# thunlp/OpenMatch

Hardware: NVIDIA H100
Metric: queries/sec top-1000 over 8.8M x 768 corpus (higher is better)
Workload: dtype f16

## Files before the change

openmatch_b200/csrc/scan_gemm.cuh:

```cuda
#pragma once
#include <cuda_fp16.h>

#include "scan_epilogue.cuh"

namespace om {

constexpr int kScanBlockN = 256;
constexpr int kScanStages = 3;
constexpr int kScanABytes = kBlockM * kBlockK * 2;
constexpr int kScanBBytes = kScanBlockN * kBlockK * 2;
constexpr int kScanStageBytes = kScanABytes + kScanBBytes;
constexpr int kScanConsumers = 256;
constexpr int kScanStash = 4;
constexpr int kScanStashOffset = kScanStages * kScanStageBytes;
constexpr int kScanStashBytes = 2 * 2 * kScanStash * kScanConsumers * 8;
constexpr int kScanBarOffset = kScanStashOffset + kScanStashBytes;
constexpr int kScanSmemBytes = kScanBarOffset + 2 * kScanStages * 8 + 1024;
static_assert(kScanSmemBytes <= 232448, "scan ring + stash exceed the 227 KB of shared memory an H100 block may use");

template <int H>
__device__ __forceinline__ float scan_pick(const float (&acc)[128], int i) {
  float a[32], b[16], c[8], d[4], e[2];
#pragma unroll
  for (int j = 0; j < 32; ++j) a[j] = (i & 1) ? acc[4 * j + 2 * H + 1] : acc[4 * j + 2 * H];
#pragma unroll
  for (int j = 0; j < 16; ++j) b[j] = (i & 2) ? a[2 * j + 1] : a[2 * j];
#pragma unroll
  for (int j = 0; j < 8; ++j) c[j] = (i & 4) ? b[2 * j + 1] : b[2 * j];
#pragma unroll
  for (int j = 0; j < 4; ++j) d[j] = (i & 8) ? c[2 * j + 1] : c[2 * j];
#pragma unroll
  for (int j = 0; j < 2; ++j) e[j] = (i & 16) ? d[2 * j + 1] : d[2 * j];
  return (i & 32) ? e[1] : e[0];
}

template <int H>
__device__ __forceinline__ int scan_filter_row(const float (&acc)[128], float t, int row, int lim, int q4, int col0,
                                               unsigned long long* stash, unsigned long long* cand, int* count,
                                               int* overflow, int C, uint32_t row_base) {
  float mx = acc[2 * H];
#pragma unroll
  for (int j = 0; j < 32; ++j) mx = fmaxf(mx, fmaxf(acc[4 * j + 2 * H], acc[4 * j + 2 * H + 1]));
  if (!(mx > t)) return 0;
  uint32_t lo = 0, hi = 0;
#pragma unroll
  for (int i = 0; i < 32; ++i) {
    lo |= (acc[4 * (i >> 1) + 2 * H + (i & 1)] > t ? 1u : 0u) << i;
    hi |= (acc[4 * (16 + (i >> 1)) + 2 * H + (i & 1)] > t ? 1u : 0u) << i;
  }
  unsigned long long mask = (static_cast<unsigned long long>(hi) << 32) | lo;
  if (lim < kScanBlockN) {
#pragma unroll 1
    for (int i = 0; i < 64; ++i)
      if (8 * (i >> 1) + 2 * q4 + (i & 1) >= lim) mask &= ~(1ull << i);
  }
  const int n = __popcll(mask);
  int pos = 0;
  if (n > kScanStash) {
    pos = atomicAdd(count + row, n - kScanStash);
    if (pos + (n - kScanStash) > C) *overflow = 1;
  }
  unsigned long long* mine = cand + static_cast<size_t>(row) * C;
  int idx = 0;
#pragma unroll 1
  while (mask) {
    const int i = __ffsll(static_cast<long long>(mask)) - 1;
    mask &= mask - 1;
    const unsigned long long key =
        make_key(scan_pick<H>(acc, i), row_base + static_cast<uint32_t>(col0 + 8 * (i >> 1) + 2 * q4 + (i & 1)));
    if (idx < kScanStash)
      stash[idx * kScanConsumers] = key;
    else if (pos + idx - kScanStash < C)
      mine[pos + idx - kScanStash] = key;
    ++idx;
  }
  return n < kScanStash ? n : kScanStash;
}

template <int CQ, int CX>
struct ScanCluster {
  static_assert((CQ == 2 || CQ == 4) && (CX == 1 || CX == 2), "scan cluster shapes: CQ in {2, 4}, CX in {1, 2}");
  static constexpr int kSize = CQ * CX;
  static constexpr int kShare = CQ + CX - 1;
  static constexpr int kQRows = kBlockM / CX;
  static constexpr int kXRows = kScanBlockN / CQ;
  static constexpr int kEmptyArrivals = kShare * (kScanConsumers / 32);
  __device__ static uint32_t peer_rank(uint32_t rank, int j) {
    const uint32_t a = rank % CQ, b = rank / CQ;
    if (j < CQ - 1) {
      const uint32_t o = static_cast<uint32_t>(j);
      return (o < a ? o : o + 1) + CQ * b;
    }
    const uint32_t o = static_cast<uint32_t>(j - (CQ - 1));
    return a + CQ * (o < b ? o : o + 1);
  }
  __device__ static uint16_t q_mask(uint32_t rank) {
    uint32_t m = 0;
#pragma unroll
    for (int b = 0; b < CX; ++b) m |= 1u << (rank % CQ + CQ * b);
    return static_cast<uint16_t>(m);
  }
  __device__ static uint16_t x_mask(uint32_t rank) {
    return static_cast<uint16_t>(((1u << CQ) - 1u) << (CQ * (rank / CQ)));
  }
};

template <int CQ, int CX>
__global__ void __launch_bounds__(kGemmProducerThreads + kScanConsumers, 1)
scan_wide_kernel(const __grid_constant__ CUtensorMap tmQ, const __grid_constant__ CUtensorMap tmX, int K,
                 const float* __restrict__ thr, unsigned long long* cand, int* count, int* overflow, int nq, int n_cols,
                 int C, uint32_t row_base) {
  using Cl = ScanCluster<CQ, CX>;
  extern __shared__ uint8_t smem_raw[];
  uint8_t* smem = reinterpret_cast<uint8_t*>((reinterpret_cast<uintptr_t>(smem_raw) + 1023) & ~uintptr_t(1023));
  unsigned long long* stash = reinterpret_cast<unsigned long long*>(smem + kScanStashOffset);
  uint64_t* full_bar = reinterpret_cast<uint64_t*>(smem + kScanBarOffset);
  uint64_t* empty_bar = full_bar + kScanStages;
  const uint32_t rank = cluster_ctarank();
  const int qa = static_cast<int>(rank % CQ), xb = static_cast<int>(rank / CQ);
  const int warp = __shfl_sync(0xffffffffu, static_cast<int>(threadIdx.x >> 5), 0);
  const int lane = static_cast<int>(threadIdx.x & 31);

  if (warp == 0 && lane == 0) {
    tma_prefetch_desc(&tmQ);
    tma_prefetch_desc(&tmX);
  }
  if (warp == 1 && lane == 0) {
    ring_init(full_bar, empty_bar, kScanStages, Cl::kEmptyArrivals);
    fence_barrier_init();
  }
  cluster_sync_all();

  const int qgroups = (nq + CQ * kBlockM - 1) / (CQ * kBlockM);
  const int num_tiles = qgroups * ((n_cols + CX * kScanBlockN - 1) / (CX * kScanBlockN));
  const int num_k = (K + kBlockK - 1) / kBlockK;

  if (warp < 4) {
    setmaxnreg_dec<40>();
    if (warp == 0 && lane == 0) {
      const uint16_t qmask = Cl::q_mask(rank), xmask = Cl::x_mask(rank);
      Ring<kScanStages> ring;
      for (int tile = static_cast<int>(cluster_id_x()); tile < num_tiles; tile += static_cast<int>(cluster_count_x())) {
        const int m_blk = (tile % qgroups) * CQ + qa;
        const int n_blk = (tile / qgroups) * CX + xb;
        for (int kb = 0; kb < num_k; ++kb) {
          uint64_t* bar = ring_acquire_tx(full_bar, empty_bar, ring, kScanStageBytes, 30);
          uint8_t* sa = smem + ring.stage * kScanStageBytes;
          if constexpr (CX == 1)
            tma_load_2d(sa, &tmQ, bar, kb * kBlockK, m_blk * kBlockM);
          else
            tma_load_2d_multicast(sa + xb * (Cl::kQRows * kBlockK * 2), &tmQ, bar, kb * kBlockK,
                                  m_blk * kBlockM + xb * Cl::kQRows, qmask);
          tma_load_2d_multicast(sa + kScanABytes + qa * (Cl::kXRows * kBlockK * 2), &tmX, bar, kb * kBlockK,
                                n_blk * kScanBlockN + qa * Cl::kXRows, xmask);
          ring.advance();
        }
      }
    }
  } else {
    setmaxnreg_inc<232>();
    const int et = static_cast<int>(threadIdx.x) - kGemmProducerThreads;
    const int wg = et >> 7;
    const int q4 = lane & 3;
    const int frow = 64 * wg + 16 * (warp & 3) + (lane >> 2);
    Ring<kScanStages> ring;
    int buf = 0;
    int p_n0 = 0, p_n1 = 0, p_excl0 = 0, p_excl1 = 0, p_pos0 = 0, p_pos1 = 0, p_row = 0, p_buf = 0;
    auto drain = [&]() {
      if (!__any_sync(0xffffffffu, (p_n0 | p_n1) != 0)) return;
      const int b0 = __shfl_sync(0xffffffffu, p_pos0, lane & ~3) + p_excl0;
      const int b1 = __shfl_sync(0xffffffffu, p_pos1, lane & ~3) + p_excl1;
      const unsigned long long* s = stash + p_buf * (2 * kScanStash * kScanConsumers) + et;
      unsigned long long* m0 = cand + static_cast<size_t>(p_row) * C;
      unsigned long long* m1 = cand + static_cast<size_t>(p_row + 8) * C;
      for (int j = 0; j < p_n0; ++j)
        if (b0 + j < C) m0[b0 + j] = s[j * kScanConsumers];
      for (int j = 0; j < p_n1; ++j)
        if (b1 + j < C) m1[b1 + j] = s[(kScanStash + j) * kScanConsumers];
      if ((p_n0 > 0 && b0 + p_n0 > C) || (p_n1 > 0 && b1 + p_n1 > C)) *overflow = 1;
      p_n0 = p_n1 = 0;
    };

    uint32_t peers[Cl::kShare - 1];
#pragma unroll
    for (int j = 0; j < Cl::kShare - 1; ++j) peers[j] = Cl::peer_rank(rank, j);
    auto release = [&](uint32_t s) {
      if (lane == 0) {
        mbar_arrive(&empty_bar[s]);
#pragma unroll
        for (int j = 0; j < Cl::kShare - 1; ++j) mbar_arrive_remote(&empty_bar[s], peers[j]);
      }
    };

    for (int tile = static_cast<int>(cluster_id_x()); tile < num_tiles; tile += static_cast<int>(cluster_count_x())) {
      const int m_blk = (tile % qgroups) * CQ + qa;
      const int n_blk = (tile / qgroups) * CX + xb;
      const int row0 = m_blk * kBlockM + frow, row1 = row0 + 8;
      const float inf = __int_as_float(0x7f800000);
      const float t0 = row0 < nq ? thr[row0] : inf, t1 = row1 < nq ? thr[row1] : inf;

      float acc[128];
#pragma unroll
      for (int i = 0; i < 128; ++i) acc[i] = 0.f;
      ring_consume(
          full_bar, ring, 0, num_k, 31,
          [&](uint32_t stage, uint32_t accumulate) {
            const uint32_t a_addr = smem_u32(smem + stage * kScanStageBytes) + wg * (64 * 128);
            const uint32_t b_addr = smem_u32(smem + stage * kScanStageBytes + kScanABytes);
#pragma unroll
            for (int k = 0; k < kBlockK / kWgmmaK; ++k)
              wgmma_m64n256k16_f16<0, 0>(acc, wgmma_desc(a_addr + k * 32, kDescKMajorSW128),
                                         wgmma_desc(b_addr + k * 32, kDescKMajorSW128), (accumulate | k) != 0 ? 1u : 0u);
          },
          release);
      wgmma_fence_regs(acc);

      drain();
      const int col0 = n_blk * kScanBlockN;
      const int lim = n_cols - col0;
      unsigned long long* sb = stash + buf * (2 * kScanStash * kScanConsumers) + et;
      const int k0 = scan_filter_row<0>(acc, t0, row0, lim, q4, col0, sb, cand, count, overflow, C, row_base);
      const int k1 = scan_filter_row<1>(acc, t1, row1, lim, q4, col0, sb + kScanStash * kScanConsumers, cand, count,
                                        overflow, C, row_base);
      if (__any_sync(0xffffffffu, (k0 | k1) != 0)) {
        int x0 = k0, x1 = k1;
        int y0 = __shfl_up_sync(0xffffffffu, x0, 1, 4), y1 = __shfl_up_sync(0xffffffffu, x1, 1, 4);
        if (q4 >= 1) x0 += y0, x1 += y1;
        y0 = __shfl_up_sync(0xffffffffu, x0, 2, 4), y1 = __shfl_up_sync(0xffffffffu, x1, 2, 4);
        if (q4 >= 2) x0 += y0, x1 += y1;
        const int n0 = __shfl_sync(0xffffffffu, x0, lane | 3), n1 = __shfl_sync(0xffffffffu, x1, lane | 3);
        if (q4 == 0) {
          if (n0 > 0) p_pos0 = atomicAdd(count + row0, n0);
          if (n1 > 0) p_pos1 = atomicAdd(count + row1, n1);
        }
        p_n0 = k0;
        p_n1 = k1;
        p_excl0 = x0 - k0;
        p_excl1 = x1 - k1;
        p_row = row0;
        p_buf = buf;
        buf ^= 1;
      }
    }
    drain();
  }

  __syncthreads();
  cluster_sync_all();
}

template <int CQ, int CX>
static inline cudaError_t scan_wide_max_clusters(int num_sms, int* out) {
  static int max_clusters = -1;
  if (max_clusters < 0) {
    constexpr int kSize = ScanCluster<CQ, CX>::kSize;
    cudaError_t e =
        cudaFuncSetAttribute(scan_wide_kernel<CQ, CX>, cudaFuncAttributeMaxDynamicSharedMemorySize, kScanSmemBytes);
    if (e != cudaSuccess) return e;
    cudaLaunchConfig_t cfg = {};
    cfg.gridDim = dim3(kSize * (num_sms / kSize));
    cfg.blockDim = dim3(kGemmProducerThreads + kScanConsumers);
    cfg.dynamicSmemBytes = kScanSmemBytes;
    cudaLaunchAttribute attr[1];
    attr[0].id = cudaLaunchAttributeClusterDimension;
    attr[0].val.clusterDim = {static_cast<unsigned>(kSize), 1, 1};
    cfg.attrs = attr;
    cfg.numAttrs = 1;
    int n = 0;
    e = cudaOccupancyMaxActiveClusters(&n, scan_wide_kernel<CQ, CX>, &cfg);
    if (e != cudaSuccess) return e;
    max_clusters = n < num_sms / kSize ? n : num_sms / kSize;
  }
  *out = max_clusters;
  return cudaSuccess;
}

template <int CQ, int CX>
static inline cudaError_t launch_scan_wide(const __half* Q, int64_t ldq, const __half* X, int64_t ldx, int nq, int n_cols,
                                           int K, const float* thr, unsigned long long* cand, int* count, int* overflow,
                                           int C, uint32_t row_base, int num_sms, cudaStream_t stream) {
  using Cl = ScanCluster<CQ, CX>;
  CUtensorMap tmQ, tmX;
  if (make_tmap_bf16_2d(&tmQ, Q, (uint64_t)K, (uint64_t)nq, (uint64_t)ldq * 2, kBlockK, Cl::kQRows) != 0)
    return cudaErrorInvalidValue;
  if (make_tmap_bf16_2d(&tmX, X, (uint64_t)K, (uint64_t)n_cols, (uint64_t)ldx * 2, kBlockK, Cl::kXRows) != 0)
    return cudaErrorInvalidValue;
  int max_clusters = 0;
  cudaError_t e = scan_wide_max_clusters<CQ, CX>(num_sms, &max_clusters);
  if (e != cudaSuccess) return e;
  if (max_clusters < 1) return cudaErrorNotSupported;
  cudaLaunchConfig_t cfg = {};
  cfg.blockDim = dim3(kGemmProducerThreads + kScanConsumers);
  cfg.dynamicSmemBytes = kScanSmemBytes;
  cfg.stream = stream;
  cudaLaunchAttribute attr[1];
  attr[0].id = cudaLaunchAttributeClusterDimension;
  attr[0].val.clusterDim = {static_cast<unsigned>(Cl::kSize), 1, 1};
  cfg.attrs = attr;
  cfg.numAttrs = 1;
  const int qgroups = (nq + CQ * kBlockM - 1) / (CQ * kBlockM);
  const int64_t num_tiles = static_cast<int64_t>(qgroups) * ((n_cols + CX * kScanBlockN - 1) / (CX * kScanBlockN));
  const int clusters = num_tiles < max_clusters ? static_cast<int>(num_tiles) : max_clusters;
  cfg.gridDim = dim3(Cl::kSize * clusters);
  return cudaLaunchKernelEx(&cfg, scan_wide_kernel<CQ, CX>, tmQ, tmX, K, thr, cand, count, overflow, nq, n_cols, C,
                            row_base);
}

static inline cudaError_t launch_scan_cluster(int cq, int cx, const __half* Q, int64_t ldq, const __half* X, int64_t ldx,
                                              int nq, int n_cols, int K, const float* thr, unsigned long long* cand,
                                              int* count, int* overflow, int C, uint32_t row_base, int num_sms,
                                              cudaStream_t stream) {
  if (nq <= 0 || n_cols <= 0 || K <= 0) return cudaSuccess;
  if (cq == 2 && cx == 1)
    return launch_scan_wide<2, 1>(Q, ldq, X, ldx, nq, n_cols, K, thr, cand, count, overflow, C, row_base, num_sms, stream);
  if (cq == 4 && cx == 1)
    return launch_scan_wide<4, 1>(Q, ldq, X, ldx, nq, n_cols, K, thr, cand, count, overflow, C, row_base, num_sms, stream);
  if (cq == 2 && cx == 2)
    return launch_scan_wide<2, 2>(Q, ldq, X, ldx, nq, n_cols, K, thr, cand, count, overflow, C, row_base, num_sms, stream);
  if (cq == 4 && cx == 2)
    return launch_scan_wide<4, 2>(Q, ldq, X, ldx, nq, n_cols, K, thr, cand, count, overflow, C, row_base, num_sms, stream);
  return cudaErrorInvalidValue;
}

static inline cudaError_t scan_cluster_capacity(int cq, int cx, int num_sms, int* out) {
  *out = -1;
  if (cq == 2 && cx == 1) return scan_wide_max_clusters<2, 1>(num_sms, out);
  if (cq == 4 && cx == 1) return scan_wide_max_clusters<4, 1>(num_sms, out);
  if (cq == 2 && cx == 2) return scan_wide_max_clusters<2, 2>(num_sms, out);
  if (cq == 4 && cx == 2) return scan_wide_max_clusters<4, 2>(num_sms, out);
  return cudaSuccess;
}

}
```

openmatch_b200/csrc/search.cu:

```cuda
#include <cuda_fp16.h>
#include <float.h>
#include <math.h>
#include <stdlib.h>
#include <string.h>

#include <algorithm>
#include <new>
#include <type_traits>
#include <vector>

#include "common.h"
#include "gemm.cuh"
#include "nccl_dyn.h"
#include "quant_i8.cuh"
#include "scan_epilogue.cuh"
#include "scan_gemm.cuh"
#include "scan_i8.cuh"

namespace om {

__device__ __forceinline__ void bitonic_sort_desc(unsigned long long* s, int P, int tid, int nthreads) {
  for (int k = 2; k <= P; k <<= 1) {
    for (int j = k >> 1; j > 0; j >>= 1) {
      for (int t = tid; t < (P >> 1); t += nthreads) {
// ... 621 lines not shown
  __half* xh = nullptr;
  int8_t* xq = nullptr;
  float* gstats = nullptr;
  bool gstats_stale = false;
  int64_t st_nonfinite = 0;
  int64_t rescore_slack = -1;
  int force_safe = 0;
  int pair_scan = 1;
  int scan_cq = 0, scan_cx = 0;
  int growth = 0;
  int certify = 1;
  int exact_only = 0;
  int stage_scores = 0;
  int64_t st_rounds = 0, st_retries = 0, st_capacity = 0, st_launches = 0;
  int64_t st_flagged = 0, st_flagged_wide = 0, st_exact = 0;
  int64_t st_scan_cluster = 0, st_scan_clusters = 0;
  int profile = 0;
  double st_scan_us = 0, st_select_us = 0, st_final_us = 0, st_other_us = 0;
  std::vector<cudaEvent_t> ev;
  std::vector<int> ev_kind;
  size_t ev_used = 0;
  DevBuf ws, ows, sws;
  int* h_status = nullptr;
};

template <typename F>
static decltype(auto) with_rows(const om_index* ix, F&& f) {
  switch (ix->storage) {
    case OM_I8: return f(ix->xq);
    case OM_F16: return f(ix->xh);
    default: return f(ix->xf);
  }
}

template <typename RowT>
static int64_t pitch_of(const RowT*, int d) { return StoredRow<RowT>::pitch(d); }

struct RowBuf {
  void** p;
  size_t row_bytes;
  const char* name;
};
template <typename RowT>
static RowBuf row_buf(RowT** p, int d, const char* name) {
  return {reinterpret_cast<void**>(p), StoredRow<RowT>::pitch(d) * sizeof(RowT), name};
}

static int index_grow(om_index* ix, int64_t need) {
  if (need <= ix->cap) return 0;
  int64_t ncap = std::max<int64_t>(need, ix->cap + ix->cap / 2);
  ncap = round_up(std::max<int64_t>(ncap, 1024), 256);
  std::vector<RowBuf> bufs;
  switch (ix->storage) {
    case OM_I8: bufs = {row_buf(&ix->xq, ix->d, "int8")}; break;
    case OM_F16: bufs = {row_buf(&ix->xh, ix->d, "fp16")}; break;
    default: bufs = {row_buf(&ix->xf, ix->d, "fp32"), row_buf(&ix->xh, ix->d, "fp16")};
  }
  void* fresh[2] = {};
  OM_CUDA(cudaDeviceSynchronize());
  for (size_t b = 0; b < bufs.size(); ++b) {
    if (dev_malloc(&fresh[b], static_cast<size_t>(ncap) * bufs[b].row_bytes) != cudaSuccess) {
      for (void* p : fresh) cudaFree(p);
      cudaGetLastError();
      return fail(OM_ENOMEM, "index: cannot allocate the %s rows for %lld rows", bufs[b].name, (long long)ncap);
    }
    if (ix->n > 0)
      OM_CUDA(cudaMemcpy(fresh[b], *bufs[b].p, static_cast<size_t>(ix->n) * bufs[b].row_bytes, cudaMemcpyDeviceToDevice));
  }
  OM_CUDA(cudaDeviceSynchronize());
  for (size_t b = 0; b < bufs.size(); ++b) {
    cudaFree(*bufs[b].p);
    *bufs[b].p = fresh[b];
  }
  ix->cap = ncap;
  return 0;
}

static inline int grid_for(int64_t n, int threads) {
  int64_t g = (n + threads - 1) / threads;
  return static_cast<int>(std::min<int64_t>(std::max<int64_t>(g, 1), 132 * 16));
}

static int settle_reset(om_index* ix, cudaStream_t st) {
  if (!ix->gstats_stale) return 0;
  OM_CUDA(cudaMemsetAsync(ix->gstats, 0, 3 * sizeof(float), st));
  ix->gstats_stale = false;
  return 0;
}

static int stage_input(const void* x, om_memkind kind, size_t bytes, cudaStream_t st, const void** src, void** tmp) {
  *src = x;
  if (kind != OM_HOST) return 0;
  OM_CUDA(cudaMalloc(tmp, bytes));
  OM_CUDA(cudaMemcpyAsync(*tmp, x, bytes, cudaMemcpyHostToDevice, st));
  *src = *tmp;
  return 0;
}

template <typename F>
static decltype(auto) with_input(const void* src, om_dtype dtype, F&& f) {
  if (dtype == OM_F32) return f(static_cast<const float*>(src));
  if (dtype == OM_BF16) return f(static_cast<const __nv_bfloat16*>(src));
  return f(static_cast<const __half*>(src));
}

extern "C" {

int om_index_create(int d, om_index** out) { return om_index_create_typed(d, OM_F32, out); }

int om_index_create_typed(int d, om_dtype storage, om_index** out) {
  if (!out || d <= 0) return fail(OM_EINVAL, "om_index_create: d must be positive");
  if (storage != OM_F32 && storage != OM_F16 && storage != OM_I8)
    return fail(OM_EINVAL, "om_index_create_typed: storage must be OM_F32, OM_F16 or OM_I8");
  OM_TRY(device_sm_count());
  om_index* ix = new (std::nothrow) om_index();
  if (!ix) return fail(OM_ENOMEM, "om_index_create: out of host memory");
  ix->d = d;
  ix->dpad = storage == OM_I8 ? i8_dpad(d) : StoredRow<__half>::pitch(d);
  ix->storage = storage;
  if (cudaMalloc(&ix->gstats, 4 * sizeof(float)) != cudaSuccess || cudaMemset(ix->gstats, 0, 4 * sizeof(float)) != cudaSuccess ||
      cudaHostAlloc(&ix->h_status, 8 * sizeof(int), cudaHostAllocDefault) != cudaSuccess) {
    cudaGetLastError();
    cudaFree(ix->gstats);
    delete ix;
    return fail(OM_ENOMEM, "om_index_create: cannot allocate index state");
  }
  *out = ix;
  return 0;
}

void om_index_destroy(om_index* ix) {
  if (!ix) return;
  cudaFree(ix->xf);
  cudaFree(ix->xh);
  cudaFree(ix->xq);
  cudaFree(ix->gstats);
  if (ix->h_status) cudaFreeHost(ix->h_status);
  ix->ws.release();
  ix->ows.release();
  ix->sws.release();
  for (cudaEvent_t e : ix->ev) cudaEventDestroy(e);
  delete ix;
}

int64_t om_index_ntotal(const om_index* ix) { return ix ? ix->n : 0; }
int om_index_dim(const om_index* ix) { return ix ? ix->d : 0; }
int om_index_storage(const om_index* ix) { return ix ? ix->storage : fail(OM_EINVAL, "om_index_storage: null index"); }

int om_index_reset(om_index* ix) {
  if (!ix) return fail(OM_EINVAL, "om_index_reset: null index");
  ix->n = 0;
  ix->gstats_stale = true;
  ix->st_nonfinite = 0;
  return 0;
}

int om_index_reserve_rows(om_index* ix, int64_t n, void** dev_rows, int64_t* row_pitch_elems) {
  if (!ix || n < 0 || !dev_rows || !row_pitch_elems) return fail(OM_EINVAL, "om_index_reserve_rows: bad arguments");
  if (ix->n + n > 0xfffffff0ll) return fail(OM_EINVAL, "index shard limited to 2^32-16 rows; shard the corpus");
  OM_TRY(index_grow(ix, ix->n + n));
  with_rows(ix, [&](auto* xs) {
    *row_pitch_elems = pitch_of(xs, ix->d);
    *dev_rows = xs + ix->n * *row_pitch_elems;
  });
  return 0;
}

int om_index_reserve(om_index* ix, int64_t n, float** dev_rows) {
  if (!ix || n < 0 || !dev_rows) return fail(OM_EINVAL, "om_index_reserve: bad arguments");
  if (ix->storage != OM_F32)
    return fail(OM_ESTATE, "om_index_reserve: the index stores %s rows; use om_index_reserve_rows",
                ix->storage == OM_F16 ? "fp16" : "int8");
  void* rows = nullptr;
  int64_t pitch = 0;
  OM_TRY(om_index_reserve_rows(ix, n, &rows, &pitch));
  *dev_rows = static_cast<float*>(rows);
  return 0;
}

int om_index_commit(om_index* ix, int64_t n, void* stream) {
  if (!ix || n < 0 || ix->n + n > ix->cap) return fail(OM_EINVAL, "om_index_commit: more rows than reserved");
  if (n == 0) return 0;
  cudaStream_t st = static_cast<cudaStream_t>(stream);
  OM_TRY(settle_reset(ix, st));
  with_rows(ix, [&](auto* xs) {
    auto* rows = xs + ix->n * pitch_of(xs, ix->d);
    if constexpr (std::is_same<decltype(rows), float*>::value)
      rows_to_f16_kernel<<<grid_for(n, 8), 256, 0, st>>>(rows, ix->xh + static_cast<size_t>(ix->n) * ix->dpad, n, ix->d,
                                                         ix->dpad, nullptr, nullptr, ix->gstats);
    else
      commit_rows_kernel<<<grid_for(n, 8), 256, 0, st>>>(rows, n, ix->d, ix->gstats, reinterpret_cast<int*>(ix->gstats) + 2);
  });
  OM_CUDA(cudaGetLastError());
  ix->n += n;
  return 0;
}

static int add_converted(om_index* ix, const void* x, om_memkind kind, om_dtype dtype, int64_t n, cudaStream_t st) {
  void* rows = nullptr;
  int64_t pitch = 0;
  OM_TRY(om_index_reserve_rows(ix, n, &rows, &pitch));
  const size_t elems = static_cast<size_t>(n) * ix->d;
  const void* src = nullptr;
  void* tmp = nullptr;
  OM_TRY(stage_input(x, kind, elems * (dtype == OM_F32 ? 4 : 2), st, &src, &tmp));
  const bool i8 = ix->storage == OM_I8;
  int* bad = reinterpret_cast<int*>(ix->gstats) + 3;
  cudaError_t e = cudaMemsetAsync(bad, 0, sizeof(int), st);
  if (e == cudaSuccess)
    e = with_input(src, dtype, [&](const auto* in) {
      if (i8)
        quantize_rows_i8_kernel<<<grid_for(n, 8), 256, 0, st>>>(in, n, ix->d, static_cast<int8_t*>(rows), pitch, bad);
      else
        to_f16_rows_kernel<<<grid_for(static_cast<int64_t>(elems), 256), 256, 0, st>>>(in, n, ix->d, static_cast<__half*>(rows),
                                                                                        ix->dpad, bad);
      return cudaGetLastError();
    });
  if (e == cudaSuccess) e = cudaMemcpyAsync(ix->h_status + 4, bad, sizeof(int), cudaMemcpyDeviceToHost, st);
  if (e == cudaSuccess) e = cudaStreamSynchronize(st);
  if (tmp) cudaFree(tmp);
  OM_CUDA(e);
  if (ix->h_status[4] > 0 && i8)
    return fail(OM_EINVAL, "om_index_add: %d rows hold inf or NaN; int8 storage cannot hold them and no row was added",
                ix->h_status[4]);
  if (ix->h_status[4] > 0)
    return fail(OM_EINVAL, "om_index_add: %d elements are NaN or round to +-inf in fp16 (|x| >= 65520); fp16 storage cannot "
                "hold them and no row was added", ix->h_status[4]);
  return om_index_commit(ix, n, st);
}

int om_index_add(om_index* ix, const void* x, om_memkind kind, om_dtype dtype, int64_t n, void* stream) {
  if (!ix || (!x && n > 0) || n < 0) return fail(OM_EINVAL, "om_index_add: bad arguments");
  if (n == 0) return 0;
  if (dtype != OM_F32 && dtype != OM_BF16 && dtype != OM_F16) return fail(OM_EINVAL, "om_index_add: unsupported dtype %d", (int)dtype);
  cudaStream_t st = static_cast<cudaStream_t>(stream);
  if (ix->storage != OM_F32) return add_converted(ix, x, kind, dtype, n, st);
  float* dst = nullptr;
  OM_TRY(om_index_reserve(ix, n, &dst));
  const size_t elems = static_cast<size_t>(n) * ix->d;
  const void* src = x;
  void* tmp = nullptr;
  if (dtype != OM_F32) OM_TRY(stage_input(x, kind, elems * 2, st, &src, &tmp));
  OM_TRY(with_input(src, dtype, [&](const auto* in) -> int {
    if constexpr (std::is_same<decltype(in), const float*>::value) {
      OM_CUDA(cudaMemcpyAsync(dst, in, elems * 4, kind == OM_HOST ? cudaMemcpyHostToDevice : cudaMemcpyDeviceToDevice, st));
    } else {
      to_f32<<<grid_for(elems, 256), 256, 0, st>>>(in, dst, (int64_t)elems);
      OM_CUDA(cudaGetLastError());
    }
    return 0;
  }));
  if (tmp) {
    OM_CUDA(cudaStreamSynchronize(st));
    cudaFree(tmp);
  }
  OM_TRY(om_index_commit(ix, n, stream));
  if (kind == OM_HOST) OM_CUDA(cudaStreamSynchronize(st));
  return 0;
}

int om_index_set_param(om_index* ix, const char* name, int64_t value) {
  if (!ix || !name) return fail(OM_EINVAL, "om_index_set_param: bad arguments");
  if (!strcmp(name, "rescore_slack")) {
    ix->rescore_slack = value;
  } else if (!strcmp(name, "force_safe_rounds")) {
    ix->force_safe = value != 0;
  } else if (!strcmp(name, "round_growth")) {
    if (value != 0 && (value < 2 || value > 8)) return fail(OM_EINVAL, "round_growth must be 0 (auto) or in [2, 8]");
    ix->growth = static_cast<int>(value);
  } else if (!strcmp(name, "pair_scan")) {
    ix->pair_scan = value != 0;
  } else if (!strcmp(name, "scan_cluster_q")) {
    if (value != 0 && value != 2 && value != 4) return fail(OM_EINVAL, "scan_cluster_q must be 0 (auto), 2 or 4");
    ix->scan_cq = static_cast<int>(value);
  } else if (!strcmp(name, "scan_cluster_x")) {
    if (value != 0 && value != 1 && value != 2) return fail(OM_EINVAL, "scan_cluster_x must be 0 (auto), 1 or 2");
    ix->scan_cx = static_cast<int>(value);
  } else if (!strcmp(name, "profile")) {
    ix->profile = static_cast<int>(value);
  } else if (!strcmp(name, "certify")) {
    ix->certify = value != 0;
  } else if (!strcmp(name, "exact_only")) {
    ix->exact_only = value != 0;
  } else if (!strcmp(name, "debug_stage_scores")) {
    ix->stage_scores = value != 0;
  } else {
    return fail(OM_EINVAL, "om_index_set_param: unknown parameter '%s'", name);
  }
  return 0;
}

int64_t om_index_get_stat(const om_index* ix, const char* name) {
  if (!ix || !name) return -1;
  if (!strcmp(name, "rounds")) return ix->st_rounds;
  if (!strcmp(name, "overflow_retries")) return ix->st_retries;
  if (!strcmp(name, "candidates")) return ix->st_capacity;
  if (!strcmp(name, "launches")) return ix->st_launches;
  if (!strcmp(name, "uncertified")) return ix->st_flagged;
  if (!strcmp(name, "uncertified_wide")) return ix->st_flagged_wide;
  if (!strcmp(name, "exact_queries")) return ix->st_exact;
  if (!strcmp(name, "nonfinite_rows")) return ix->st_nonfinite;
  if (!strcmp(name, "scan_cluster")) return ix->st_scan_cluster;
  if (!strcmp(name, "scan_max_clusters")) return ix->st_scan_clusters;
  if (!strcmp(name, "scan_ns")) return static_cast<int64_t>(ix->st_scan_us * 1e3);
  if (!strcmp(name, "select_ns")) return static_cast<int64_t>(ix->st_select_us * 1e3);
  if (!strcmp(name, "finalize_ns")) return static_cast<int64_t>(ix->st_final_us * 1e3);
  if (!strcmp(name, "other_ns")) return static_cast<int64_t>(ix->st_other_us * 1e3);
  return -1;
}

}

namespace {

struct Timed {
  om_index* ix;
  cudaStream_t st;
  bool on;
  Timed(om_index* ix_, cudaStream_t st_, int kind) : ix(ix_), st(st_), on(ix_->profile != 0) {
    static const char* nvtx_names[4] = {"om.search.scan", "om.search.select", "om.search.rescore", "om.search.exchange_certify"};
    nvtxRangePushA(nvtx_names[kind & 3]);
    if (!on) return;
    if (ix->ev_used + 2 > ix->ev.size()) {
      cudaEvent_t a, b;
      if (cudaEventCreate(&a) != cudaSuccess || cudaEventCreate(&b) != cudaSuccess) {
        on = false;
        return;
      }
      ix->ev.push_back(a);
      ix->ev.push_back(b);
      ix->ev_kind.push_back(0);
    }
    ix->ev_kind[ix->ev_used / 2] = kind;
    cudaEventRecord(ix->ev[ix->ev_used], st);
  }
  ~Timed() {
    nvtxRangePop();
    if (!on) return;
    cudaEventRecord(ix->ev[ix->ev_used + 1], st);
    ix->ev_used += 2;
  }
};

void collect_profile(om_index* ix) {
  static const char* names[4] = {"scan", "select", "finalize", "exchange+certify"};
  for (size_t i = 0; i + 1 < ix->ev_used; i += 2) {
    float ms = 0.f;
    if (cudaEventElapsedTime(&ms, ix->ev[i], ix->ev[i + 1]) != cudaSuccess) continue;
    const int kind = ix->ev_kind[i / 2];
    (kind == 0 ? ix->st_scan_us : kind == 1 ? ix->st_select_us : kind == 2 ? ix->st_final_us : ix->st_other_us) += ms * 1e3;
    if (ix->profile >= 2) fprintf(stderr, "[om profile] launch %zu %s %.3f ms\n", i / 2, names[kind & 3], ms);
  }
  ix->ev_used = 0;
}

int once_attrs(const om_index* ix) {
  static bool done = false;
  if (!done) {
    OM_CUDA(cudaFuncSetAttribute(select_kernel, cudaFuncAttributeMaxDynamicSharedMemorySize, 16384 * 8));
    OM_CUDA(cudaFuncSetAttribute(merge_kernel, cudaFuncAttributeMaxDynamicSharedMemorySize, 8192 * 16));
    done = true;
  }
  return !ix ? 0 : with_rows(ix, [](const auto* xs) -> int {
    using RowT = std::decay_t<decltype(*xs)>;
    static bool rows_done = false;
    if (rows_done) return 0;
    OM_CUDA(cudaFuncSetAttribute(finalize_kernel<RowT>, cudaFuncAttributeMaxDynamicSharedMemorySize, kMaxCandidates * 8 + 65536));
    OM_CUDA(cudaFuncSetAttribute(exact_scan_kernel<8, 2, RowT>, cudaFuncAttributeMaxDynamicSharedMemorySize, 96 * 1024));
    rows_done = true;
    return 0;
  });
}

struct ExchangeBlock {
  size_t off_i, off_floor, off_stats, bytes;
};
inline ExchangeBlock exchange_block(size_t nqc, size_t kc) {
  ExchangeBlock b;
  b.off_i = round_up(nqc * kc * 4, 256);
  b.off_floor = b.off_i + round_up(nqc * kc * 8, 256);
  b.off_stats = b.off_floor + round_up(nqc * 4, 256);
  b.bytes = b.off_stats + 256;
  return b;
}
inline size_t exchange_block_bytes(size_t nqc, size_t kc) { return exchange_block(nqc, kc).bytes; }

int level_prepare(om_index* ix, Level& L, const float* qf, int nq, int k, int kp_target, int mode, int world,
                  cudaStream_t st) {
  const int d = ix->d, dpad = ix->dpad;
  if (d > 16384) return fail(OM_EINVAL, "om_index_search: d > 16384 unsupported");
  if (k > kMaxCandidates) return fail(OM_EINVAL, "om_index_search: k = %d exceeds %d", k, kMaxCandidates);
  OM_TRY(once_attrs(ix));
  L.qf = qf;
  L.nq = nq;
  L.k = k;
  L.mode = mode;
  L.world = world;
  L.kp_target = std::min(std::max(kp_target, k), kMaxCandidates);
  if (world > 1 && mode == 0 && L.kp_target < kMaxCandidates) {
    const double m = static_cast<double>(L.kp_target) / world;
    L.kp_target = static_cast<int>(std::min<int64_t>(L.kp_target, round_up(static_cast<int64_t>(m + 6.0 * sqrt(m) + 32.0), 32)));
  }
  L.kp = static_cast<int>(std::min<int64_t>(L.kp_target, std::max<int64_t>(ix->n, 1)));
  for (L.growth = ix->growth > 0 ? ix->growth : (nq <= 256 ? 8 : 2);; --L.growth) {
    L.C = 1024;
    while (L.C < (5 * L.growth * L.kp) / 4 + 512) L.C <<= 1;
    if (L.C <= 16384 || L.growth == 2) break;
  }
  if (L.C > 16384) return fail(OM_EINVAL, "om_index_search: candidate list of %d entries exceeds 16384; lower k", L.C);
  L.kc = std::min(k, L.kp_target);
  L.nqc_max = std::min(nq, kQueryChunk);
  ix->st_capacity = L.C;
  size_t off = 0;
  auto carve = [&](size_t bytes) {
    size_t o = off;
    off += round_up(bytes, 256);
    return o;
  };
  const size_t nqc = L.nqc_max;
  const size_t o_qh = carve(static_cast<size_t>(nq) * dpad * 2), o_hn = carve(static_cast<size_t>(nq) * 4),
               o_en = carve(static_cast<size_t>(nq) * 4), o_cand = carve(nqc * L.C * 8), o_count = carve(nqc * 4),
               o_thr = carve(nqc * 4), o_status = carve(256), o_sig = carve(static_cast<size_t>(nq) * 8);
  size_t o_send = 0, o_recv = 0;
  if (world > 1) {
    const size_t blk = exchange_block_bytes(nqc, L.kc);
    o_send = carve(blk);
    o_recv = carve(blk * world);
  }
  OM_TRY(ix->ws.reserve(off));
  uint8_t* base = static_cast<uint8_t*>(ix->ws.p);
  L.qh = reinterpret_cast<__half*>(base + o_qh);
  L.q8 = reinterpret_cast<int8_t*>(base + o_qh);
  L.qsig = reinterpret_cast<float2*>(base + o_sig);
  L.hn = reinterpret_cast<float*>(base + o_hn);
  L.en = reinterpret_cast<float*>(base + o_en);
  L.cand = reinterpret_cast<unsigned long long*>(base + o_cand);
  L.count = reinterpret_cast<int*>(base + o_count);
  L.thr = reinterpret_cast<float*>(base + o_thr);
  L.status = reinterpret_cast<int*>(base + o_status);
  L.send = world > 1 ? base + o_send : nullptr;
  L.recv = world > 1 ? base + o_recv : nullptr;
  if (mode == 0 && ix->storage == OM_I8) {
    queries_to_i8_kernel<<<grid_for(nq, 8), 256, 0, st>>>(qf, nq, d, dpad, L.q8, L.q8 + static_cast<size_t>(nq) * dpad, L.qsig,
                                                          L.hn, L.en);
    OM_CUDA(cudaGetLastError());
    ix->st_launches += 1;
  } else if (mode == 0) {
    rows_to_f16_kernel<<<grid_for(nq, 8), 256, 0, st>>>(qf, L.qh, nq, d, dpad, L.hn, L.en, nullptr);
    OM_CUDA(cudaGetLastError());
    ix->st_launches += 1;
  }
  return 0;
}

int sweep_chunk(om_index* ix, const Level& L, int q0, int nqc, bool safe, int sms, cudaStream_t st) {
  const int64_t growth = L.growth;
  const int64_t N = ix->n;
  const int C = L.C, kp = L.kp;
  if (N == 0) {
    fill_i32<<<(nqc + 255) / 256, 256, 0, st>>>(L.count, 0, nqc);
    fill_i32<<<(nqc + 255) / 256, 256, 0, st>>>(reinterpret_cast<int*>(L.thr), static_cast<int>(0xff800000), nqc);
    OM_CUDA(cudaGetLastError());
    return 0;
  }
  const __half* qh = L.qh + static_cast<size_t>(q0) * ix->dpad;
  const float* qf = L.qf + static_cast<size_t>(q0) * ix->d;
  int* overflow = L.status;
  int64_t pos = 0;
  const size_t sel_smem = static_cast<size_t>(C) * 8;
  bool first = true;
  while (pos < N) {
    int64_t step;
    if (first)
      step = std::min<int64_t>(N, C);
    else if (safe)
      step = std::min<int64_t>(N - pos, std::max<int64_t>(256, ((C - kp) / 256) * 256));
    else
      step = std::min<int64_t>(N - pos, (growth - 1) * pos);
    {
      Timed t(ix, st, 0);
      if (L.mode == 0 && ix->storage == OM_I8) {
        const int8_t* qhi = L.q8 + static_cast<size_t>(q0) * ix->dpad;
        const int8_t* qlo = L.q8 + (static_cast<size_t>(L.nq) + q0) * ix->dpad;
        const int64_t pitch = pitch_of(ix->xq, ix->d);
        const int8_t* xrows = ix->xq + pos * pitch;
        const int ncols = static_cast<int>(step);
        cudaError_t e;
        if (first)
          e = launch_scan_i8<true>(qhi, qlo, ix->dpad, L.qsig + q0, xrows, pitch, ix->dpad, nqc, ncols, ix->d, L.thr,
                                   L.cand, L.count, overflow, C, static_cast<uint32_t>(pos), sms, st);
        else
          e = launch_scan_i8<false>(qhi, qlo, ix->dpad, L.qsig + q0, xrows, pitch, ix->dpad, nqc, ncols, ix->d, L.thr,
                                    L.cand, L.count, overflow, C, static_cast<uint32_t>(pos), sms, st);
        if (e != cudaSuccess) return fail(OM_ECUDA, "int8 scan kernel launch failed: %s", cudaGetErrorString(e));
      } else if (L.mode == 0) {
        const __half* xrows = ix->xh + static_cast<size_t>(pos) * ix->dpad;
        cudaError_t e;
        const int ncols = static_cast<int>(step);
        const bool pair = ix->pair_scan != 0 && nqc > kBlockM;
        if (first) {
          EpiScan<true> epi{L.thr, L.cand, L.count, overflow, nqc, ncols, C, static_cast<uint32_t>(pos)};
          e = launch_gemm<128, 3, true, EpiScan<true>, true>(qh, ix->dpad, xrows, ix->dpad, nqc, ncols, ix->d, epi, sms, st, true);
        } else if (pair) {
          const int cq = ix->scan_cq ? ix->scan_cq : 2, cx = ix->scan_cx ? ix->scan_cx : 1;
          int clusters = 0;
          e = launch_scan_cluster(cq, cx, qh, ix->dpad, xrows, ix->dpad, nqc, ncols, ix->d, L.thr, L.cand, L.count,
                                  overflow, C, static_cast<uint32_t>(pos), sms, st);
          if (e == cudaSuccess) e = scan_cluster_capacity(cq, cx, sms, &clusters);
          ix->st_scan_cluster = 10 * cq + cx;
          ix->st_scan_clusters = clusters;
        } else {
          EpiScan<false> epi{L.thr, L.cand, L.count, overflow, nqc, ncols, C, static_cast<uint32_t>(pos)};
          e = launch_gemm<128, 3, true, EpiScan<false>, true>(qh, ix->dpad, xrows, ix->dpad, nqc, ncols, ix->d, epi, sms, st, true);
        }
        if (e != cudaSuccess) return fail(OM_ECUDA, "scan kernel launch failed: %s", cudaGetErrorString(e));
      } else {
        const int nqt = std::max(1, std::min(8, (96 * 1024) / (ix->d * 4)));
        dim3 grid(static_cast<unsigned>(std::min<int64_t>((step + 15) / 16, static_cast<int64_t>(sms) * 4)),
                  static_cast<unsigned>((nqc + nqt - 1) / nqt));
        const size_t smem = static_cast<size_t>(nqt) * ix->d * 4;
        with_rows(ix, [&](const auto* xs) {
          exact_scan_kernel<8, 2><<<grid, 256, smem, st>>>(xs + pos * pitch_of(xs, ix->d), step, static_cast<uint32_t>(pos), qf,
                                                           nqc, ix->d, nqt, L.thr, L.cand, L.count, overflow, C, first ? 1 : 0);
        });
        OM_CUDA(cudaGetLastError());
      }
    }
    {
      Timed t(ix, st, 1);
      select_kernel<<<nqc, 256, sel_smem, st>>>(L.cand, L.count, L.thr, C, kp, first ? static_cast<int>(step) : -1);
    }
    OM_CUDA(cudaGetLastError());
    ix->st_launches += 2;
    pos += step;
    first = false;
    ix->st_rounds++;
  }
  return 0;
}

int finalize_chunk(om_index* ix, const Level& L, int q0, int nqc, float* D, int64_t* I, int k_out, int64_t id_offset,
                   cudaStream_t st) {
  int P2 = 2;
  while (P2 < L.kp) P2 <<= 1;
  const size_t fin_smem = static_cast<size_t>(P2) * 8 + static_cast<size_t>(ix->d) * 4;
  {
    Timed t(ix, st, 2);
    const float* qf = L.qf + static_cast<size_t>(q0) * ix->d;
    with_rows(ix, [&](const auto* xs) {
      finalize_kernel<<<nqc, 256, fin_smem, st>>>(L.cand, L.count, L.C, qf, xs, ix->d, D, I, id_offset, k_out,
                                                  ix->stage_scores);
    });
  }
  OM_CUDA(cudaGetLastError());
  ix->st_launches += 1;
  return 0;
}

#define OM_NCCL(expr)                                                                                   \
  do {                                                                                                  \
    int r__ = (expr);                                                                                   \
    if (r__ != 0) return fail(OM_ECUDA, "%s failed: %s", #expr, nccl_api().GetErrorString(r__));        \
  } while (0)

int merge_parts(const float* Dp, const int64_t* Ip, int64_t stride_d, int64_t stride_i, int nparts, int nq, int k_in,
                int k_out, float* D, int64_t* I, cudaStream_t st) {
  OM_TRY(once_attrs(nullptr));
  if (k_in > 8192) return fail(OM_EINVAL, "om_topk_merge_n: k_in = %d exceeds 8192", k_in);
  if (static_cast<int64_t>(nparts) * k_in <= 8192) {
    int P = 2;
    while (P < nparts * k_in) P <<= 1;
    const size_t smem = static_cast<size_t>(P) * 8 + static_cast<size_t>(nparts) * k_in * 8;
    merge_kernel<<<nq, 256, smem, st>>>(Dp, Ip, stride_d, stride_i, nparts, nq, k_in, k_out, D, I);
    OM_CUDA(cudaGetLastError());
    return 0;
  }
  if (k_in > 4096 || k_out > 4096)
    return fail(OM_EINVAL, "om_topk_merge_n: %d parts x %d entries exceed one merge of 8192 and need k_in, k_out <= 4096 "
                "(got k_in = %d, k_out = %d)", nparts, k_in, k_in, k_out);
  const int g = std::max(2, 8192 / k_in);
  const int ngroups = (nparts + g - 1) / g;
  const int k_mid = static_cast<int>(std::min<int64_t>(k_out, static_cast<int64_t>(g) * k_in));
  float* Dm = nullptr;
  int64_t* Im = nullptr;
  const size_t per = static_cast<size_t>(nq) * k_mid;
  OM_CUDA(cudaMallocAsync(&Dm, per * ngroups * 4, st));
  OM_CUDA(cudaMallocAsync(&Im, per * ngroups * 8, st));
  int rc = 0;
  for (int gi = 0; gi < ngroups && rc == 0; ++gi) {
    const int p0 = gi * g, np = std::min(g, nparts - p0);
    rc = merge_parts(Dp + p0 * stride_d, Ip + p0 * stride_i, stride_d, stride_i, np, nq, k_in, k_mid, Dm + gi * per,
                     Im + gi * per, st);
  }
  if (rc == 0) rc = merge_parts(Dm, Im, static_cast<int64_t>(per), static_cast<int64_t>(per), ngroups, nq, k_mid, k_out, D, I, st);
  cudaFreeAsync(Dm, st);
  cudaFreeAsync(Im, st);
  return rc;
}

int exchange_chunk(om_index* ix, om_comm* comm, const Level& L, int q0, int nqc, float* dD, int64_t* dI, int64_t id_offset,
                   cudaStream_t st) {
  NcclApi& nc = nccl_api();
  const int W = comm->world;
  const ExchangeBlock b = exchange_block(nqc, L.kc);
  OM_TRY(finalize_chunk(ix, L, q0, nqc, reinterpret_cast<float*>(L.send), reinterpret_cast<int64_t*>(L.send + b.off_i), L.kc,
                        id_offset, st));
// ... 257 lines not shown
```

Baseline: 38080.

## Drop producer warps, widen scan tile to three consumer warpgroups with inline TMA issue

Removes the dedicated producer warpgroup and has consumer thread 0 issue TMA loads from the release callback, tracked through shared-memory loader state. Each CTA now covers 192 query rows with three warpgroups of 384 threads, which cuts re-streaming of the corpus tile per query group and adds compute per loaded X tile. The risks are that load issue becomes serialized behind consumer progress, which hurts overlap, and that the register budget shifts: setmaxnreg is gone, so 384 threads share 64K registers and hold 128-float accumulators, which may cause spills. Shared memory per stage also grows.

Measured after the change: 38240 (median of 6 runs). Within noise of the previous version (+0.4%).

```diff
diff --git a/openmatch_b200/csrc/scan_gemm.cuh b/openmatch_b200/csrc/scan_gemm.cuh
--- a/openmatch_b200/csrc/scan_gemm.cuh
+++ b/openmatch_b200/csrc/scan_gemm.cuh
@@ -5,12 +5,13 @@
 
 namespace om {
 
+constexpr int kScanBlockM = 192;
 constexpr int kScanBlockN = 256;
 constexpr int kScanStages = 3;
-constexpr int kScanABytes = kBlockM * kBlockK * 2;
+constexpr int kScanABytes = kScanBlockM * kBlockK * 2;
 constexpr int kScanBBytes = kScanBlockN * kBlockK * 2;
 constexpr int kScanStageBytes = kScanABytes + kScanBBytes;
-constexpr int kScanConsumers = 256;
+constexpr int kScanConsumers = 384;
 constexpr int kScanStash = 4;
 constexpr int kScanStashOffset = kScanStages * kScanStageBytes;
 constexpr int kScanStashBytes = 2 * 2 * kScanStash * kScanConsumers * 8;
@@ -82,7 +83,7 @@
   static_assert((CQ == 2 || CQ == 4) && (CX == 1 || CX == 2), "scan cluster shapes: CQ in {2, 4}, CX in {1, 2}");
   static constexpr int kSize = CQ * CX;
   static constexpr int kShare = CQ + CX - 1;
-  static constexpr int kQRows = kBlockM / CX;
+  static constexpr int kQRows = kScanBlockM / CX;
   static constexpr int kXRows = kScanBlockN / CQ;
   static constexpr int kEmptyArrivals = kShare * (kScanConsumers / 32);
   __device__ static uint32_t peer_rank(uint32_t rank, int j) {
@@ -106,7 +107,7 @@
 };
 
 template <int CQ, int CX>
-__global__ void __launch_bounds__(kGemmProducerThreads + kScanConsumers, 1)
+__global__ void __launch_bounds__(kScanConsumers, 1)
 scan_wide_kernel(const __grid_constant__ CUtensorMap tmQ, const __grid_constant__ CUtensorMap tmX, int K,
                  const float* __restrict__ thr, unsigned long long* cand, int* count, int* overflow, int nq, int n_cols,
                  int C, uint32_t row_base) {
@@ -121,129 +122,132 @@
   const int warp = __shfl_sync(0xffffffffu, static_cast<int>(threadIdx.x >> 5), 0);
   const int lane = static_cast<int>(threadIdx.x & 31);
 
-  if (warp == 0 && lane == 0) {
+  if (threadIdx.x == 0) {
     tma_prefetch_desc(&tmQ);
     tma_prefetch_desc(&tmX);
-  }
-  if (warp == 1 && lane == 0) {
     ring_init(full_bar, empty_bar, kScanStages, Cl::kEmptyArrivals);
     fence_barrier_init();
   }
   cluster_sync_all();
 
-  const int qgroups = (nq + CQ * kBlockM - 1) / (CQ * kBlockM);
+  const int qgroups = (nq + CQ * kScanBlockM - 1) / (CQ * kScanBlockM);
   const int num_tiles = qgroups * ((n_cols + CX * kScanBlockN - 1) / (CX * kScanBlockN));
   const int num_k = (K + kBlockK - 1) / kBlockK;
 
-  if (warp < 4) {
-    setmaxnreg_dec<40>();
-    if (warp == 0 && lane == 0) {
-      const uint16_t qmask = Cl::q_mask(rank), xmask = Cl::x_mask(rank);
-      Ring<kScanStages> ring;
-      for (int tile = static_cast<int>(cluster_id_x()); tile < num_tiles; tile += static_cast<int>(cluster_count_x())) {
-        const int m_blk = (tile % qgroups) * CQ + qa;
-        const int n_blk = (tile / qgroups) * CX + xb;
-        for (int kb = 0; kb < num_k; ++kb) {
-          uint64_t* bar = ring_acquire_tx(full_bar, empty_bar, ring, kScanStageBytes, 30);
-          uint8_t* sa = smem + ring.stage * kScanStageBytes;
-          if constexpr (CX == 1)
-            tma_load_2d(sa, &tmQ, bar, kb * kBlockK, m_blk * kBlockM);
-          else
-            tma_load_2d_multicast(sa + xb * (Cl::kQRows * kBlockK * 2), &tmQ, bar, kb * kBlockK,
-                                  m_blk * kBlockM + xb * Cl::kQRows, qmask);
-          tma_load_2d_multicast(sa + kScanABytes + qa * (Cl::kXRows * kBlockK * 2), &tmX, bar, kb * kBlockK,
-                                n_blk * kScanBlockN + qa * Cl::kXRows, xmask);
-          ring.advance();
-        }
+  __shared__ struct {
+    int tile, kb, q_row, x_row;
+    uint32_t stage, phase;
+  } ld;
+  auto seek = [&](int tile) {
+    ld.tile = tile;
+    ld.kb = 0;
+    ld.q_row = ((tile % qgroups) * CQ + qa) * kScanBlockM + xb * Cl::kQRows;
+    ld.x_row = ((tile / qgroups) * CX + xb) * kScanBlockN + qa * Cl::kXRows;
+  };
+  auto load_next = [&]() {
+    if (ld.tile >= num_tiles) return;
+    Ring<kScanStages> r;
+    r.stage = ld.stage;
+    r.phase = ld.phase;
+    uint64_t* bar = ring_acquire_tx(full_bar, empty_bar, r, kScanStageBytes, 30);
+    uint8_t* sa = smem + r.stage * kScanStageBytes;
+    if constexpr (CX == 1)
+      tma_load_2d(sa, &tmQ, bar, ld.kb * kBlockK, ld.q_row);
+    else
+      tma_load_2d_multicast(sa + xb * (Cl::kQRows * kBlockK * 2), &tmQ, bar, ld.kb * kBlockK, ld.q_row,
+                            Cl::q_mask(rank));
+    tma_load_2d_multicast(sa + kScanABytes + qa * (Cl::kXRows * kBlockK * 2), &tmX, bar, ld.kb * kBlockK, ld.x_row,
+                          Cl::x_mask(rank));
+    r.advance();
+    ld.stage = r.stage;
+    ld.phase = r.phase;
+    if (++ld.kb == num_k) seek(ld.tile + static_cast<int>(cluster_count_x()));
+  };
+  if (threadIdx.x == 0) {
+    ld.stage = ld.phase = 0;
+    seek(static_cast<int>(cluster_id_x()));
+    for (int s = 0; s < kScanStages; ++s) load_next();
+  }
+
+  const int et = static_cast<int>(threadIdx.x);
+  const int wg = et >> 7;
+  const int q4 = lane & 3;
+  const int frow = 64 * wg + 16 * (warp & 3) + (lane >> 2);
+  Ring<kScanStages> ring;
+  int buf = 0;
+  int p_cnt = 0, p_pos0 = 0, p_pos1 = 0, p_row = 0;
+  auto drain = [&]() {
+    if (!__any_sync(0xffffffffu, (p_cnt & 0xffff) != 0)) return;
+    const int n0 = p_cnt & 0xff, n1 = (p_cnt >> 8) & 0xff;
+    const int b0 = __shfl_sync(0xffffffffu, p_pos0, lane & ~3) + ((p_cnt >> 16) & 0xff);
+    const int b1 = __shfl_sync(0xffffffffu, p_pos1, lane & ~3) + (p_cnt >> 24);
+    const unsigned long long* s = stash + (buf ^ 1) * (2 * kScanStash * kScanConsumers) + et;
+    unsigned long long* m0 = cand + static_cast<size_t>(p_row) * C;
+    unsigned long long* m1 = cand + static_cast<size_t>(p_row + 8) * C;
+    for (int j = 0; j < n0; ++j)
+      if (b0 + j < C) m0[b0 + j] = s[j * kScanConsumers];
+    for (int j = 0; j < n1; ++j)
+      if (b1 + j < C) m1[b1 + j] = s[(kScanStash + j) * kScanConsumers];
+    if ((n0 > 0 && b0 + n0 > C) || (n1 > 0 && b1 + n1 > C)) *overflow = 1;
+    p_cnt = 0;
+  };
+
+  auto release = [&](uint32_t s) {
+    if (lane == 0) {
+      mbar_arrive(&empty_bar[s]);
+#pragma unroll 1
+      for (int j = 0; j < Cl::kShare - 1; ++j) mbar_arrive_remote(&empty_bar[s], Cl::peer_rank(rank, j));
+      if (warp == 0) load_next();
+    }
+    __syncwarp();
+  };
+
+  for (int tile = static_cast<int>(cluster_id_x()); tile < num_tiles; tile += static_cast<int>(cluster_count_x())) {
+    const int m_blk = (tile % qgroups) * CQ + qa;
+    const int n_blk = (tile / qgroups) * CX + xb;
+    const int row0 = m_blk * kScanBlockM + frow, row1 = row0 + 8;
+    const float inf = __int_as_float(0x7f800000);
+    const float t0 = row0 < nq ? thr[row0] : inf, t1 = row1 < nq ? thr[row1] : inf;
+    float acc[128];
+#pragma unroll
+    for (int i = 0; i < 128; ++i) acc[i] = 0.f;
+    ring_consume(
+        full_bar, ring, 0, num_k, 31,
+        [&](uint32_t stage, uint32_t accumulate) {
+          const uint32_t a_addr = smem_u32(smem + stage * kScanStageBytes) + wg * (64 * 128);
+          const uint32_t b_addr = smem_u32(smem + stage * kScanStageBytes + kScanABytes);
+#pragma unroll
+          for (int k = 0; k < kBlockK / kWgmmaK; ++k)
+            wgmma_m64n256k16_f16<0, 0>(acc, wgmma_desc(a_addr + k * 32, kDescKMajorSW128),
+                                       wgmma_desc(b_addr + k * 32, kDescKMajorSW128), (accumulate | k) != 0 ? 1u : 0u);
+        },
+        release);
+    wgmma_fence_regs(acc);
+
+    drain();
+    const int col0 = n_blk * kScanBlockN;
+    const int lim = n_cols - col0;
+    unsigned long long* sb = stash + buf * (2 * kScanStash * kScanConsumers) + et;
+    const int k0 = scan_filter_row<0>(acc, t0, row0, lim, q4, col0, sb, cand, count, overflow, C, row_base);
+    const int k1 = scan_filter_row<1>(acc, t1, row1, lim, q4, col0, sb + kScanStash * kScanConsumers, cand, count,
+                                      overflow, C, row_base);
+    if (__any_sync(0xffffffffu, (k0 | k1) != 0)) {
+      int x0 = k0, x1 = k1;
+      int y0 = __shfl_up_sync(0xffffffffu, x0, 1, 4), y1 = __shfl_up_sync(0xffffffffu, x1, 1, 4);
+      if (q4 >= 1) x0 += y0, x1 += y1;
+      y0 = __shfl_up_sync(0xffffffffu, x0, 2, 4), y1 = __shfl_up_sync(0xffffffffu, x1, 2, 4);
+      if (q4 >= 2) x0 += y0, x1 += y1;
+      const int n0 = __shfl_sync(0xffffffffu, x0, lane | 3), n1 = __shfl_sync(0xffffffffu, x1, lane | 3);
+      if (q4 == 0) {
+        if (n0 > 0) p_pos0 = atomicAdd(count + row0, n0);
+        if (n1 > 0) p_pos1 = atomicAdd(count + row1, n1);
       }
+      p_cnt = k0 | k1 << 8 | (x0 - k0) << 16 | (x1 - k1) << 24;
+      p_row = row0;
+      buf ^= 1;
     }
-  } else {
-    setmaxnreg_inc<232>();
-    const int et = static_cast<int>(threadIdx.x) - kGemmProducerThreads;
-    const int wg = et >> 7;
-    const int q4 = lane & 3;
-    const int frow = 64 * wg + 16 * (warp & 3) + (lane >> 2);
-    Ring<kScanStages> ring;
-    int buf = 0;
-    int p_n0 = 0, p_n1 = 0, p_excl0 = 0, p_excl1 = 0, p_pos0 = 0, p_pos1 = 0, p_row = 0, p_buf = 0;
-    auto drain = [&]() {
-      if (!__any_sync(0xffffffffu, (p_n0 | p_n1) != 0)) return;
-      const int b0 = __shfl_sync(0xffffffffu, p_pos0, lane & ~3) + p_excl0;
-      const int b1 = __shfl_sync(0xffffffffu, p_pos1, lane & ~3) + p_excl1;
-      const unsigned long long* s = stash + p_buf * (2 * kScanStash * kScanConsumers) + et;
-      unsigned long long* m0 = cand + static_cast<size_t>(p_row) * C;
-      unsigned long long* m1 = cand + static_cast<size_t>(p_row + 8) * C;
-      for (int j = 0; j < p_n0; ++j)
-        if (b0 + j < C) m0[b0 + j] = s[j * kScanConsumers];
-      for (int j = 0; j < p_n1; ++j)
-        if (b1 + j < C) m1[b1 + j] = s[(kScanStash + j) * kScanConsumers];
-      if ((p_n0 > 0 && b0 + p_n0 > C) || (p_n1 > 0 && b1 + p_n1 > C)) *overflow = 1;
-      p_n0 = p_n1 = 0;
-    };
-
-    uint32_t peers[Cl::kShare - 1];
-#pragma unroll
-    for (int j = 0; j < Cl::kShare - 1; ++j) peers[j] = Cl::peer_rank(rank, j);
-    auto release = [&](uint32_t s) {
-      if (lane == 0) {
-        mbar_arrive(&empty_bar[s]);
-#pragma unroll
-        for (int j = 0; j < Cl::kShare - 1; ++j) mbar_arrive_remote(&empty_bar[s], peers[j]);
-      }
-    };
-
-    for (int tile = static_cast<int>(cluster_id_x()); tile < num_tiles; tile += static_cast<int>(cluster_count_x())) {
-      const int m_blk = (tile % qgroups) * CQ + qa;
-      const int n_blk = (tile / qgroups) * CX + xb;
-      const int row0 = m_blk * kBlockM + frow, row1 = row0 + 8;
-      const float inf = __int_as_float(0x7f800000);
-      const float t0 = row0 < nq ? thr[row0] : inf, t1 = row1 < nq ? thr[row1] : inf;
-
-      float acc[128];
-#pragma unroll
-      for (int i = 0; i < 128; ++i) acc[i] = 0.f;
-      ring_consume(
-          full_bar, ring, 0, num_k, 31,
-          [&](uint32_t stage, uint32_t accumulate) {
-            const uint32_t a_addr = smem_u32(smem + stage * kScanStageBytes) + wg * (64 * 128);
-            const uint32_t b_addr = smem_u32(smem + stage * kScanStageBytes + kScanABytes);
-#pragma unroll
-            for (int k = 0; k < kBlockK / kWgmmaK; ++k)
-              wgmma_m64n256k16_f16<0, 0>(acc, wgmma_desc(a_addr + k * 32, kDescKMajorSW128),
-                                         wgmma_desc(b_addr + k * 32, kDescKMajorSW128), (accumulate | k) != 0 ? 1u : 0u);
-          },
-          release);
-      wgmma_fence_regs(acc);
-
-      drain();
-      const int col0 = n_blk * kScanBlockN;
-      const int lim = n_cols - col0;
-      unsigned long long* sb = stash + buf * (2 * kScanStash * kScanConsumers) + et;
-      const int k0 = scan_filter_row<0>(acc, t0, row0, lim, q4, col0, sb, cand, count, overflow, C, row_base);
-      const int k1 = scan_filter_row<1>(acc, t1, row1, lim, q4, col0, sb + kScanStash * kScanConsumers, cand, count,
-                                        overflow, C, row_base);
-      if (__any_sync(0xffffffffu, (k0 | k1) != 0)) {
-        int x0 = k0, x1 = k1;
-        int y0 = __shfl_up_sync(0xffffffffu, x0, 1, 4), y1 = __shfl_up_sync(0xffffffffu, x1, 1, 4);
-        if (q4 >= 1) x0 += y0, x1 += y1;
-        y0 = __shfl_up_sync(0xffffffffu, x0, 2, 4), y1 = __shfl_up_sync(0xffffffffu, x1, 2, 4);
-        if (q4 >= 2) x0 += y0, x1 += y1;
-        const int n0 = __shfl_sync(0xffffffffu, x0, lane | 3), n1 = __shfl_sync(0xffffffffu, x1, lane | 3);
-        if (q4 == 0) {
-          if (n0 > 0) p_pos0 = atomicAdd(count + row0, n0);
-          if (n1 > 0) p_pos1 = atomicAdd(count + row1, n1);
-        }
-        p_n0 = k0;
-        p_n1 = k1;
-        p_excl0 = x0 - k0;
-        p_excl1 = x1 - k1;
-        p_row = row0;
-        p_buf = buf;
-        buf ^= 1;
-      }
-    }
-    drain();
-  }
+  }
+  drain();
 
   __syncthreads();
   cluster_sync_all();
@@ -259,7 +263,7 @@
     if (e != cudaSuccess) return e;
     cudaLaunchConfig_t cfg = {};
     cfg.gridDim = dim3(kSize * (num_sms / kSize));
-    cfg.blockDim = dim3(kGemmProducerThreads + kScanConsumers);
+    cfg.blockDim = dim3(kScanConsumers);
     cfg.dynamicSmemBytes = kScanSmemBytes;
     cudaLaunchAttribute attr[1];
     attr[0].id = cudaLaunchAttributeClusterDimension;
@@ -290,7 +294,7 @@
   if (e != cudaSuccess) return e;
   if (max_clusters < 1) return cudaErrorNotSupported;
   cudaLaunchConfig_t cfg = {};
-  cfg.blockDim = dim3(kGemmProducerThreads + kScanConsumers);
+  cfg.blockDim = dim3(kScanConsumers);
   cfg.dynamicSmemBytes = kScanSmemBytes;
   cfg.stream = stream;
   cudaLaunchAttribute attr[1];
@@ -298,7 +302,7 @@
   attr[0].val.clusterDim = {static_cast<unsigned>(Cl::kSize), 1, 1};
   cfg.attrs = attr;
   cfg.numAttrs = 1;
-  const int qgroups = (nq + CQ * kBlockM - 1) / (CQ * kBlockM);
+  const int qgroups = (nq + CQ * kScanBlockM - 1) / (CQ * kScanBlockM);
   const int64_t num_tiles = static_cast<int64_t>(qgroups) * ((n_cols + CX * kScanBlockN - 1) / (CX * kScanBlockN));
   const int clusters = num_tiles < max_clusters ? static_cast<int>(num_tiles) : max_clusters;
   cfg.gridDim = dim3(Cl::kSize * clusters);
diff --git a/openmatch_b200/csrc/search.cu b/openmatch_b200/csrc/search.cu
--- a/openmatch_b200/csrc/search.cu
+++ b/openmatch_b200/csrc/search.cu
@@ -947,6 +947,7 @@
   if (!strcmp(name, "nonfinite_rows")) return ix->st_nonfinite;
   if (!strcmp(name, "scan_cluster")) return ix->st_scan_cluster;
   if (!strcmp(name, "scan_max_clusters")) return ix->st_scan_clusters;
+  if (!strcmp(name, "scan_box_queries")) return kScanBlockM;
   if (!strcmp(name, "scan_ns")) return static_cast<int64_t>(ix->st_scan_us * 1e3);
   if (!strcmp(name, "select_ns")) return static_cast<int64_t>(ix->st_select_us * 1e3);
   if (!strcmp(name, "finalize_ns")) return static_cast<int64_t>(ix->st_final_us * 1e3);
```
